# lynet55/robotic-mpc

Measured on AMD Instinct MI355X. Metric: MPC-steps/sec (whole node), UR10 N=100 dt=0.01 batch; 1/2/4/8 GPU, higher is better.
Workload: dtype f64

## Files before the change

### robotic_mpc_amd/csrc/mpc_core.h

```cpp
#pragma once
#include "mpc_kin.h"
#include "mpc_ipm.h"
#include "mpc_nlp.h"

#define MPC_REP16(X) X(0) X(1) X(2) X(3) X(4) X(5) X(6) X(7) X(8) X(9) X(10) X(11) X(12) X(13) X(14) X(15)
#define MPC_REP4(X) X(0) X(1) X(2) X(3)

namespace mpcb {

constexpr double BOUND_INF = 1e29;

constexpr int L1 = 98;
constexpr int L2N = 62;
constexpr int L2W = 114;

#ifndef MPCB_FUSE
#define MPCB_FUSE 1
#endif
#ifdef MPCB_PROFILE
#define PROF_T0(v) const double v = ex.clock()
#define PROF_ADD(i, v) prof[i] += ex.clock() - v
#else
#define PROF_T0(v)
#define PROF_ADD(i, v)
// ... 591 lines not shown
                        }
                    });
                }
                ex.par([&](int lane) {
                    ex.put_max(sm.red[0], lane, a_s.at(lane)); ex.put_max(sm.red[1], lane, a_e.at(lane));
                    ex.put_max(sm.red[2], lane, a_i.at(lane)); ex.put_max(sm.red[3], lane, a_c.at(lane));
                });
                rs = fmax(rs, ex.get_max(sm.red[0]));
                re = fmax(re, ex.get_max(sm.red[1]));
                ri = fmax(ri, ex.get_max(sm.red[2]));
                rc = fmax(rc, ex.get_max(sm.red[3]));
            }
            copies([&](int lane, auto nl) {
                constexpr int NL = decltype(nl)::value;
                if (wide) copy_lanes<W2, 0, W2, L2W, false, NL>(v2, ex.smem().w.G2, k0, k1, lane);
                else copy_lanes<W2_LIN, 0, W2, L2N, false, NL>(v2, ex.smem().w.G2, k0, k1, lane);
            });
            PROF_ADD(PF_X3, tn);
        }
        if (res4) { res4[0] = rs; res4[1] = re; res4[2] = ri; res4[3] = rc; }
        PROF_ADD(PF_NLP, t0);
        return cost;
    }

    MPC_PASS void residual_direct(int mode, double a)
    {
        PROF_T0(t0);
        Smem &sm = ex.smem();
        const InstParams &P = sm.P;
        const int Nl = ex.uni(ex.smem().n_hor), NS = Nl + 1;
        double *const G1 = ex.smem().w.G1, *const G2 = ex.smem().w.G2, *const G3 = ex.smem().w.G3;
        double *const Y = ex.pool();
        a = ex.uni(a);
        typename Ex::template PerLane<double> n_g, n_b, n_d, n_m, n_mu, n_c;
        PROF_T0(tx);
        ex.wpar([&](int lane) { n_g.at(lane) = 0; n_b.at(lane) = 0; n_d.at(lane) = 0; n_m.at(lane) = 0; n_mu.at(lane) = 0; n_c.at(lane) = 0; });
        if (mode == 1) {
            constexpr int IPS = 15, R = rounds_for(IPS);
            const int items = NS * IPS;
            for (int base = 0; base < items; base += R * NT) {
                ex.wpar([&](int lane) {
                    D2 cur[R], stp[R];
#pragma unroll
                    for (int r = 0; r < R; r++) {
                        const int e = imin(base + r * NT + lane, items - 1), k = e / IPS, c = 2 * (e - k * IPS);
                        cur[r] = *(MPC_GLOBAL const D2 *)(G1 + (size_t)k * W1 + O_QW + c);
                        stp[r] = *(MPC_GLOBAL const D2 *)(G3 + (size_t)(c >= 18 ? imin(k + 1, Nl) : k) * W3 + O_DW + c);
                    }
#pragma unroll
                    for (int r = 0; r < R; r++) {
                        const int e = base + r * NT + lane;
                        if (e < items) {
                            const int k = e / IPS, c = 2 * (e - k * IPS);
                            const double aa = (c >= 18 && k >= Nl) ? 0.0 : a;
                            D2 v = cur[r];
                            v.x += aa * stp[r].x; v.y += aa * stp[r].y;
                            *(MPC_GLOBAL D2 *)(G1 + (size_t)k * W1 + O_QW + c) = v;
                        }
                    }
                });
            }
        } else {
            ex.wpar([&](int lane) {
                if (lane < NX) gst(G1 + O_QW + 6 + lane, sm.xhat[lane] - gld(G1 + O_X + lane));
                if (lane >= 16 && lane < 16 + NU) gst(G1 + (size_t)Nl * W1 + O_QW + lane - 16, 0.0);
            });
        }
        {
            constexpr int IPS = 24, R = rounds_for(IPS);
            const int items = NS * IPS;
            for (int base = 0; base < items; base += R * NT) {
                ex.wpar([&](int lane) {
                    D2 cur[R], stp[R];
#pragma unroll
                    for (int r = 0; r < R; r++) {
                        const int e = imin(base + r * NT + lane, items - 1), k = e / IPS, q = 2 * (e - k * IPS);
                        cur[r] = *(MPC_GLOBAL const D2 *)(G1 + (size_t)k * W1 + O_QLAM + q);
                        if (mode == 1) stp[r] = *(MPC_GLOBAL const D2 *)(G3 + (size_t)k * W3 + O_DLAM + q);
                    }
                    double ncl = n_c.at(lane);
#pragma unroll
                    for (int r = 0; r < R; r++) {
                        const int e = base + r * NT + lane;
                        if (e < items) {
                            const int k = e / IPS, q = 2 * (e - k * IPS);
                            const bool is_t = q >= 24;
                            const int sc = is_t ? q - 24 : q, j = sc < 12 ? sc : sc - 12;
                            const bool ok = j < 6 ? k < Nl : (k >= 1 && k < Nl);
                            const D2 m = *reinterpret_cast<const D2 *>(&sm.bon[sc]);
                            const bool on0 = ok && m.x != 0.0, on1 = ok && m.y != 0.0;
                            D2 v = cur[r];
                            if (mode == 1) {
                                v.x = ipm::step_floor(on0, v.x, a, stp[r].x); v.y = ipm::step_floor(on1, v.y, a, stp[r].y);
                            } else {
                                v.x = is_t ? ipm::warm_t(on0, v.x) : ipm::warm_lam(on0, v.x);
                                v.y = is_t ? ipm::warm_t(on1, v.y) : ipm::warm_lam(on1, v.y);
                                ncl += (on0 && !is_t ? 1.0 : 0.0) + (on1 && !is_t ? 1.0 : 0.0);
                            }
                            *(MPC_GLOBAL D2 *)(G1 + (size_t)k * W1 + O_QLAM + q) = v;
                        }
                    }
                    n_c.at(lane) = ncl;
                });
            }
        }
        ex.barrier();
        PROF_ADD(PF_X1, tx);
        PROF_T0(ty);
        const int CY = ex.uni(imax(1, imin(ex.smem().pool_n / 6, NS)));
        for (int y0 = 0; y0 < NS; y0 += CY) {
        const int y1 = imin(y0 + CY, NS);
        if (y0 > 0) ex.barrier();
        {
            constexpr int R = rounds_for(NTASK);
            const int items = (imin(y1, Nl) - y0) * NTASK;
            for (int base = 0; base < items; base += R * NT) {
                ex.wpar([&](int lane) {
                    double g[R][12], d[R][12], rr[R];
#pragma unroll
                    for (int r = 0; r < R; r++) {
                        const int e = imax(imin(base + r * NT + lane, items - 1), 0), k = y0 + e / NTASK, i = e - (k - y0) * NTASK;
                        const double *g1 = G1 + (size_t)k * W1 + O_QW, *g2 = G2 + (size_t)k * W2;
                        rr[r] = gld(g2 + O_R + i);
#pragma unroll
                        for (int j = 0; j < 6; j++) { g[r][j] = gld(g2 + O_GQ + i * 6 + j); d[r][j] = gld(g1 + 6 + j); }
                        if (i == 4) {
#pragma unroll
                            for (int j = 0; j < 6; j++) { g[r][6 + j] = gld(g2 + O_GV + j); d[r][6 + j] = gld(g1 + 12 + j); }
                        }
                    }
#pragma unroll
                    for (int r = 0; r < R; r++) {
                        const int e = base + r * NT + lane;
                        if (e < items) {
                            const int k = y0 + e / NTASK, i = e - (k - y0) * NTASK;
                            double v = rr[r];
#pragma unroll
                            for (int j = 0; j < 6; j++) v += g[r][j] * d[r][j];
                            if (i == 4) {
#pragma unroll
                                for (int j = 0; j < 6; j++) v += g[r][6 + j] * d[r][6 + j];
                            }
                            v *= P.w_task[i];
                            Y[(k - y0) * 6 + i] = v;
                            gst(G2 + (size_t)k * W2 + O_Y + i, v);
                        }
                    }
                });
            }
        }
        ex.barrier();
        PROF_ADD(PF_X2, ty);
        PROF_T0(tz);
        {
            constexpr int R = Ex::VGPR_BUDGET <= 256 && rounds_for(6) > 2 ? 2 : rounds_for(6);
            const int items = (y1 - y0) * 6;
            const double dt = P.dt, lm = P.lm;
            auto bounds = [&](int lane, int k, int ci, double val_, double dv, double l_lo, double l_hi, double t_lo, double t_hi,
                              double &rg) {
                const bool hc = ci < 6 ? k < Nl : (k >= 1 && k < Nl);
                const bool blo = hc && sm.bon[ci] != 0.0, bhi = hc && sm.bon[12 + ci] != 0.0;
                const double val = hc ? val_ : 0.0;
                const double ll = blo ? l_lo : 0.0, lu = bhi ? l_hi : 0.0;
                const double itl = fast_rcp(t_lo), itu = fast_rcp(t_hi);
                const double rdl = blo ? dv - (bnd_lo(P, ci) - val) - t_lo : 0.0;
                const double rdu = bhi ? (bnd_hi(P, ci) - val) - dv - t_hi : 0.0;
                const double rml = ll * t_lo, rmu = lu * t_hi;
                double gt = rg;
                rg -= ll; gt -= ll;
                double gam = ll * itl;
                gt += (rml + ll * rdl) * itl;
                rg += lu; gt += lu;
                gam += lu * itu;
                gt -= (rmu + lu * rdu) * itu;
                n_mu.at(lane) += rml + rmu;
                n_d.at(lane) = fmax(n_d.at(lane), fmax(fabs(rdl), fabs(rdu)));
                n_m.at(lane) = fmax(n_m.at(lane), fmax(fabs(rml), fabs(rmu)));
                double *g3 = G3 + (size_t)k * W3, *g2 = G2 + (size_t)k * W2;
                gst(g3 + O_RD + ci, rdl); gst(g3 + O_RD + 12 + ci, rdu);
                gst(g3 + O_RM + ci, rml); gst(g3 + O_RM + 12 + ci, rmu);
                gst(g2 + O_GAM + ci, gam);
                return gt;
            };
            constexpr int RD = 2 * R;
            const int items_d = (y1 - y0) * NX;
            for (int base = 0; base < items; base += R * NT) {
                ex.wpar([&](int lane) {
                    double v[R][12], q[R][13], d[RD][5];
#pragma unroll
                    for (int r = 0; r < R; r++) {
                        const int e = imin(base + r * NT + lane, items - 1), k = y0 + e / 6, j = e - (k - y0) * 6, km = imax(k - 1, 0);
                        const double *g1 = G1 + (size_t)k * W1, *g2 = G2 + (size_t)k * W2, *gm = G1 + (size_t)km * W1;
                        v[r][0] = gld(g1 + O_U + j);      v[r][1] = gld(g1 + O_X + 6 + j);
                        v[r][2] = gld(g1 + O_QW + j);     v[r][3] = gld(g1 + O_QW + 12 + j);
                        v[r][4] = gld(g1 + O_QPI + j);    v[r][5] = gld(g1 + O_QPI + 6 + j);
                        v[r][6] = gld(gm + O_QPI + 6 + j);
                        v[r][7] = gld(g2 + O_GV + j);
                        v[r][8] = gld(g1 + O_QLAM + j);   v[r][9] = gld(g1 + O_QLAM + 12 + j);
                        v[r][10] = gld(g1 + O_QT + j);    v[r][11] = gld(g1 + O_QT + 12 + j);
                        q[r][0] = gld(g1 + O_X + j);  q[r][1] = gld(g1 + O_QW + 6 + j);
#pragma unroll
                        for (int i = 0; i < NTASK; i++) q[r][2 + i] = gld(g2 + O_GQ + i * 6 + j);
                        q[r][7] = v[r][4]; q[r][8] = gld(gm + O_QPI + j);
                        q[r][9] = gld(g1 + O_QLAM + 6 + j);  q[r][10] = gld(g1 + O_QLAM + 18 + j);
                        q[r][11] = gld(g1 + O_QT + 6 + j);   q[r][12] = gld(g1 + O_QT + 18 + j);
                    }
#pragma unroll
                    for (int r = 0; r < RD; r++) {
                        const int e = imin(2 * base + r * NT + lane, items_d - 1), k = y0 + e / NX, i = e - (k - y0) * NX, kn = imin(k + 1, Nl);
                        const double *dw = G1 + (size_t)k * W1 + O_QW;
                        d[r][0] = gld(dw + 6 + i);
                        d[r][1] = gld(dw + (i < 6 ? 12 + i : i - 6));
                        d[r][2] = gld(dw + (i < 6 ? i : i - 6));
                        d[r][3] = gld(G2 + (size_t)k * W2 + O_BD + i);
                        d[r][4] = gld(G1 + (size_t)kn * W1 + O_QW + 6 + i);
                    }
#pragma unroll
                    for (int r = 0; r < R; r++) {
                        const int e = base + r * NT + lane;
                        if (e < items) {
                            const int k = y0 + e / 6, j = e - (k - y0) * 6;
                            const double du = v[r][2], dvv = v[r][3];
                            const double uj = v[r][0] + du, vj = v[r][1] + dvv;
                            const double c2 = P.w_qddot * P.cq[j] * P.cq[j];
                            double *g3 = G3 + (size_t)k * W3, *g2 = G2 + (size_t)k * W2;
                            double rgu = 0.0;
                            if (k < Nl) {
                                rgu = dt * (2.0 * P.w_u * uj + c2 * (uj - vj));
                                rgu += P.b1[j] * v[r][4] + P.b2[j] * v[r][5];
                                rgu += dt * lm * du;
                            }
                            const double gtu = bounds(lane, k, j, v[r][0], du, v[r][8], v[r][9], v[r][10], v[r][11], rgu);
                            gst(g3 + O_RG + j, rgu); gst(g2 + O_GT + j, gtu);
                            double rgv = 0.0;
                            if (k >= 1) {
                                if (k < Nl) {
                                    rgv = dt * (v[r][7] * Y[(k - y0) * 6 + 4] + c2 * (vj - uj));
                                    rgv += P.a12[j] * v[r][4] + P.a22[j] * v[r][5];
                                }
                                rgv += (k < Nl ? dt : 1.0) * lm * dvv;
                                rgv -= v[r][6];
                            }
                            gst(g3 + O_RG + 12 + j, rgv); gst(g2 + O_GT + 12 + j, rgv);
                            const double dq = q[r][1];
                            double rg = 0.0;
                            if (k >= 1) {
                                if (k < Nl) {
                                    double s_ = 0.0;
#pragma unroll
                                    for (int i = 0; i < NTASK; i++) s_ += q[r][2 + i] * Y[(k - y0) * 6 + i];
                                    rg = dt * s_ + q[r][7];
                                }
                                rg += (k < Nl ? dt : 1.0) * lm * dq;
                                rg -= q[r][8];
                            }
                            const double gt = bounds(lane, k, 6 + j, q[r][0], dq, q[r][9], q[r][10], q[r][11], q[r][12], rg);
                            gst(g3 + O_RG + 6 + j, rg); gst(g2 + O_GT + 6 + j, gt);
                            n_g.at(lane) = fmax(n_g.at(lane), fmax(fmax(fabs(rgu), fabs(rgv)), fabs(rg)));
                        }
                    }
#pragma unroll
                    for (int r = 0; r < RD; r++) {
                        const int e = 2 * base + r * NT + lane;
                        if (e < items_d && e < 2 * (base + R * NT)) {
                            const int k = y0 + e / NX, i = e - (k - y0) * NX;
                            double vv = 0.0;
                            if (k < Nl) {
                                if (i < 6) vv = d[r][0] + P.a12[i] * d[r][1] + P.b1[i] * d[r][2];
                                else vv = P.a22[i - 6] * d[r][0] + P.b2[i - 6] * d[r][1];
                                vv += d[r][3] - d[r][4];
                                n_b.at(lane) = fmax(n_b.at(lane), fabs(vv));
                            }
                            gst(G2 + (size_t)k * W2 + O_RB + i, vv);
                        }
                    }
                });
            }
        }
        PROF_ADD(PF_X3, tz);
        }
        ex.par([&](int lane) {
            ex.put_max(sm.red[0], lane, n_g.at(lane)); ex.put_max(sm.red[1], lane, n_b.at(lane));
            ex.put_max(sm.red[2], lane, n_d.at(lane)); ex.put_max(sm.red[3], lane, n_m.at(lane));
            ex.put_sum(sm.red[4], lane, n_mu.at(lane)); ex.put_sum(sm.red[5], lane, n_c.at(lane));
        });
        const double ng = ex.get_max(sm.red[0]), nb = ex.get_max(sm.red[1]), nd = ex.get_max(sm.red[2]), nm = ex.get_max(sm.red[3]);
        const double smu = ex.get_sum(sm.red[4]), nc = ex.get_sum(sm.red[5]);
        ex.par([&](int lane) {
            if ((lane & (WAVE - 1)) == 0) {
                sm.ret[0] = ng; sm.ret[1] = nb; sm.ret[2] = nd; sm.ret[3] = nm; sm.ret[4] = smu;
                if (mode == 0) sm.ret[5] = nc;
            }
        });
        PROF_ADD(PF_RES, t0);
    }

    struct FactLane {
        double b1a, b2a, b1b, b2b, a12a, a22a, a12b, a22b;
        double hu_c;
        double huv_c;
        double lm_c;
        double mqq, mqv, mvq, mvv;
        double qqq, qqv, qvq, qvv;
        int a, b;
        int oqq, oqv, ovv;
    };

    template <int MODE>
    MPC_PASS void fact_pass_t()
    {
        constexpr bool RES = MODE == 1, SEG = MODE == 2;
        PROF_T0(t0);
        Smem &sm = ex.smem();
        const InstParams &P = sm.P;
        const int Nl = ex.uni(ex.smem().n_hor);
        constexpr int WR = 78;
        constexpr int WF = RES ? W4 - O_PM : W4;
        constexpr int FO = RES ? O_PM : 0;
        const ResMap rm = res_map();
        const int CH = RES ? chunk_len_in(rm.scr_n, 2 * (WR + WF), 2 * WR) : chunk_len(2 * (WR + W4), 2 * WR);
        typename Ex::template PerLane<FactLane> fl;
        ex.seq([&](int lane) {
            FactLane &f = fl.at(lane);
            const int a = lane < 36 ? lane / 6 : 0, b = lane < 36 ? lane % 6 : 0;
            f.a = a; f.b = b;
            f.oqq = tri(imin(a, b), imax(a, b)); f.oqv = tri(a, 6 + b); f.ovv = tri(6 + imin(a, b), 6 + imax(a, b));
            f.b1a = P.b1[a]; f.b2a = P.b2[a]; f.b1b = P.b1[b]; f.b2b = P.b2[b];
            f.a12a = P.a12[a]; f.a22a = P.a22[a]; f.a12b = P.a12[b]; f.a22b = P.a22[b];
            const double c2 = P.dt * P.w_qddot * P.cq[a] * P.cq[a];
            f.hu_c = a == b ? P.dt * 2.0 * P.w_u + c2 + P.dt * P.lm : 0.0;
            f.huv_c = a == b ? c2 : 0.0;
            f.lm_c = a == b ? P.dt * P.lm : 0.0;
            f.mqq = f.mqv = f.mvq = f.mvv = 0.0;
            f.qqq = f.qqv = f.qvq = f.qvv = 0.0;
        });
        const double dw0 = P.dt * P.w_task[0], dw1 = P.dt * P.w_task[1], dw2 = P.dt * P.w_task[2], dw3 = P.dt * P.w_task[3],
                     dw4 = P.dt * P.w_task[4];
        auto next_stage = [&](int lane, FactLane &f, double gam_u, int sb) {
            const double fq = f.b1a * f.mqq + f.b2a * f.mvq, fv = f.b1a * f.mqv + f.b2a * f.mvv;
            double r = fq * f.b1b + fv * f.b2b + f.hu_c;
            r += f.a == f.b ? gam_u : 0.0;
            sm.Rt[f.a * 6 + f.b] = r;
            double *St = sm.St2[sb];
            St[f.a * 12 + f.b] = fq;
            St[f.a * 12 + 6 + f.b] = fq * f.a12b + fv * f.a22b - f.huv_c;
            const double cq = f.a12a * f.mqq + f.a22a * f.mvq, cv = f.a12a * f.mqv + f.a22a * f.mvv;
            f.qqq = f.mqq;
            f.qqv = f.mqq * f.a12b + f.mqv * f.a22b;
            f.qvq = cq;
            f.qvv = cq * f.a12b + cv * f.a22b;
            (void)lane;
        };
        int sb = 0;
        const size_t buf = (size_t)(CH + 1) * WR + (size_t)CH * WF;
        auto vr_of = [&](int ci) { return ex.pool() + (size_t)(ci & 1) * buf; };
        auto vf_of = [&](int ci) { return vr_of(ci) + (size_t)(CH + 1) * WR; };
        auto k1_of = [&](int ci) { return Nl - ci * CH; };
        typename Ex::template PerLane<double> pr;
        typename Ex::template PerLane<double> tr, wr;
        typename Ex::template PerLane<D2> ab;
        double b1r[6], b2r[6], a12r[6], a22r[6];
#pragma unroll
        for (int i = 0; i < 6; i++) { b1r[i] = P.b1[i]; b2r[i] = P.b2[i]; a12r[i] = P.a12[i]; a22r[i] = P.a22[i]; }
        typename Ex::template PerLane<double> phi[12];
        int vcur = 0;
        auto vec_sweep = [&](int ci) {
            const int k1c = k1_of(ci), k0c = imax(k1c - CH + 1, 0), klc = imax(k0c - 1, 0);
            const double *vr = vr_of(ci);
            double *vf = vf_of(ci);
            for (int k = k1c; k >= k0c; k--) {
                const double *ric = vr + (size_t)(k - klc) * WR;
                const double *gt = ric + 48, *rbv = ric + 66;
                double *fac = vf + (size_t)(k - k0c) * WF - FO;
                double *kk = RES ? rm.K + (size_t)k * 72 : fac + O_K, *vhp = RES ? rm.VH + (size_t)k * 6 : fac + O_VH;
                double *ep = RES ? rm.E + (size_t)k * 12 : fac + O_E, *pvp = RES ? rm.P + (size_t)k * 12 : fac + O_PV;
                const double *Pn = (k < k1c ? fac + WF : vf_of(ci + 1) - FO) + O_PM;
                const int vnxt = vcur ^ 1;
                ex.await(&sm.prog, Nl - k);
                if (k == Nl) {
                    ex.sub([&](int lane) {
                        if (lane < NX) {
                            const double v = gt[6 + lane];
                            pr.at(lane) = v; ex.share(sm.pv[vcur], lane, v);
                            pvp[lane] = v; fac[O_WV + lane] = 0.0; ep[lane] = 0.0;
                            const int j = lane % 6;
                            D2 c2; c2.x = P.a12[j]; c2.y = P.a22[j];
                            ab.at(lane) = c2;
                        }
                        if (lane < NU) vhp[lane] = 0.0;
                        if (lane == 0) ex.post(&sm.prog1, 0);
                    });
                    continue;
                }
                ex.sub([&](int lane) {
                    double t = 0.0, w = 0.0;
                    if (lane < NX) {
                        double w0 = 0.0, w1 = 0.0;
#pragma unroll
                        for (int j = 0; j < NX; j += 2) { w0 += Pn[tri_sym(lane, j)] * rbv[j]; w1 += Pn[tri_sym(lane, j + 1)] * rbv[j + 1]; }
                        w = w0 + w1;
                        t = pr.at(lane) + w;
                    }
                    tr.at(lane) = t; wr.at(lane) = w;
                    ex.share(sm.mt2[vcur], lane < NX ? lane : NX, t);
                });
                ex.sub([&](int lane) {
                    const double t = tr.at(lane), w = wr.at(lane);
                    double tv[12];
#pragma unroll
                    for (int i = 0; i < NX; i++) tv[i] = ex.gather(sm.mt2[vcur], i, t);
                    const double oq = ex.shr6(sm.mt2[vcur], lane, t);
                    if (lane < NX) {
                        const int j = lane;
                        double hu[6];
#pragma unroll
                        for (int m = 0; m < 6; m++) hu[m] = gt[m] + b1r[m] * tv[m] + b2r[m] * tv[6 + m];
                        const D2 c2 = ab.at(lane);
                        double pj = gt[6 + j] + (j < 6 ? t : c2.x * oq + c2.y * t);
                        double s0 = 0.0, s1 = 0.0;
#pragma unroll
                        for (int m = 0; m < 6; m += 2) { s0 += kk[m * 12 + j] * hu[m]; s1 += kk[(m + 1) * 12 + j] * hu[m + 1]; }
                        pj -= s0 + s1;
                        pr.at(lane) = pj; ex.share(sm.pv[vnxt], lane, pj);
                        pvp[j] = pj;
                        fac[O_WV + j] = w;
                        const int i6 = j < 6 ? j : j - 6;
                        double v0 = 0.0, v1 = 0.0;
#pragma unroll
                        for (int m = 0; m < 6; m += 2) { v0 += fac[O_RI + i6 * 6 + m] * hu[m]; v1 += fac[O_RI + i6 * 6 + m + 1] * hu[m + 1]; }
                        const double vh = v0 + v1;
                        if (j < 6) vhp[j] = vh;
                        ep[j] = rbv[j] - (j < 6 ? P.b1[i6] : P.b2[i6]) * vh;
                    }
                    if (lane == 0) ex.post(&sm.prog1, Nl - k);
                });
                vcur = vnxt;
            }
        };
        constexpr int NBW = Ex::BG_WAVES;
        ex.par([&](int lane) {
            if (lane == 0) { ex.post(&sm.prog, -1); ex.post(&sm.prog1, -1); ex.post(&sm.flg[0], NBW); ex.post(&sm.flg[1], 0); }
        });
        load_rect<WR, O_GQ, W2>(vr_of(0), ex.smem().w.G2, imax(imax(Nl - CH + 1, 0) - 1, 0), Nl);
        const int nwin = (Nl + CH) / CH;
        PROF_T0(ts);
        ex.pipeline3(nwin, [&](int ci) {
            const int k1 = k1_of(ci), k0 = imax(k1 - CH + 1, 0), kl = imax(k0 - 1, 0);
            double *vr = vr_of(ci), *vf = vf_of(ci);
            ex.await(&sm.flg[0], NBW * (ci + 1));
            if (ci >= 2) ex.await(&sm.flg[1], NBW * ci);
            for (int k = k1; k >= k0; k--) {
                const double *ric = vr + (size_t)(k - kl) * WR;
                const double *ricd = ric - WR;
                double *fac = vf + (size_t)(k - k0) * WF - FO;
                double *kk = RES ? rm.K + (size_t)k * 72 : fac + O_K;
                const double *gam = ric + 36;
                if (k == Nl) {
                    ex.seq([&](int lane) {
                        const double lmN = ex.smem().P.lm;
                        for (int e = lane; e < NPM; e += WAVE) {
                            double v = 0.0;
#pragma unroll
                            for (int i = 0; i < NX; i++) v = e == tri(i, i) ? lmN : v;
                            fac[O_PM + e] = v;
                        }
                        if (lane < 36) {
                            FactLane &f = fl.at(lane);
                            f.mqv = f.mvq = 0.0;
                            f.mqq = f.mvv = f.a == f.b ? lmN : 0.0;
                            next_stage(lane, f, ricd[36 + f.a], sb);
                        }
                        if (lane == 0) ex.post(&sm.prog, 0);
                    });
                    continue;
                }
#ifndef MPCB_DIAG_NO_B
                ex.seq([&](int lane) {
                    const double *St = sm.St2[sb];
                    double A_[6][6];
#pragma unroll
                    for (int i = 0; i < 6; i++)
#pragma unroll
                        for (int j = 0; j <= i; j++) A_[i][j] = sm.Rt[i * 6 + j];
                    double dinv[6];
#pragma unroll
                    for (int j = 0; j < 6; j++) {
#ifdef MPCB_DIAG_NO_LDL
                        dinv[j] = A_[j][j]; continue;
#endif
                        dinv[j] = fast_rcp(A_[j][j]);
                        double lj[6];
#pragma unroll
                        for (int i = j + 1; i < 6; i++) lj[i] = A_[i][j] * dinv[j];
#pragma unroll
                        for (int i = j + 1; i < 6; i++)
#pragma unroll
                            for (int r = j + 1; r <= i; r++) A_[i][r] -= lj[i] * A_[r][j];
#pragma unroll
                        for (int i = j + 1; i < 6; i++) A_[i][j] = lj[i];
                    }
                    if (lane < 18) {
                        double x[6];
                        const int col = lane < 12 ? lane : 0;
#pragma unroll
                        for (int i = 0; i < 6; i++) x[i] = St[i * 12 + col];
#pragma unroll
                        for (int i = 0; i < 6; i++) x[i] = lane < 12 ? x[i] : (i == lane - 12 ? 1.0 : 0.0);
#pragma unroll
                        for (int j = 0; j < 6; j++) {
#pragma unroll
                            for (int i = j + 1; i < 6; i++) x[i] -= A_[i][j] * x[j];
                        }
#pragma unroll
                        for (int i = 0; i < 6; i++) x[i] *= dinv[i];
#pragma unroll
                        for (int j = 5; j >= 0; j--) {
#pragma unroll
                            for (int i = 0; i < j; i++) x[i] -= A_[j][i] * x[j];
                        }
                        if (lane < 12) {
#pragma unroll
                            for (int i = 0; i < 6; i++) kk[i * 12 + lane] = x[i];
                        } else {
#pragma unroll
                            for (int i = 0; i < 6; i++) fac[O_RI + i * 6 + (lane - 12)] = x[i];
                        }
                    }
                });
#endif
                ex.seq([&](int lane) {
#ifdef MPCB_DIAG_NO_CA
                    if (lane == 0) ex.post(&sm.prog, Nl - k);
                    return;
#endif
                    if (lane < 36) {
                        FactLane &f = fl.at(lane);
                        if (k > 0) {
                            const double *St = sm.St2[sb];
                            const double *gq = ric, *gv = ric + 30;
                            const double ga0 = gq[f.a], ga1 = gq[6 + f.a], ga2 = gq[12 + f.a], ga3 = gq[18 + f.a], ga4 = gq[24 + f.a];
                            const double gb0 = gq[f.b], gb1 = gq[6 + f.b], gb2 = gq[12 + f.b], gb3 = gq[18 + f.b], gb4 = gq[24 + f.b];
                            const double gva = gv[f.a], gvb = gv[f.b];
                            const double gam_q = gam[6 + f.a], gam_u = ricd[36 + f.a];
                            double sa[6], sva[6], kb[6], kvb[6];
#pragma unroll
                            for (int m = 0; m < 6; m++) { sa[m] = St[m * 12 + f.a]; sva[m] = St[m * 12 + 6 + f.a]; }
#pragma unroll
                            for (int m = 0; m < 6; m++) { kb[m] = kk[m * 12 + f.b]; kvb[m] = kk[m * 12 + 6 + f.b]; }
#if defined(__HIP_DEVICE_COMPILE__)
                            asm volatile("" ::: "memory");
#endif
                            double pqq = f.qqq + (dw0 * ga0 * gb0 + dw1 * ga1 * gb1 + dw2 * ga2 * gb2 + dw3 * ga3 * gb3 + dw4 * ga4 * gb4) + f.lm_c;
                            double pqv = f.qqv + dw4 * ga4 * gvb;
                            double pvq = f.qvq + dw4 * gva * gb4;
                            double pvv = f.qvv + dw4 * gva * gvb + (f.huv_c + f.lm_c);
                            pqq += f.a == f.b ? gam_q : 0.0;
#pragma unroll
                            for (int m = 0; m < 6; m++) {
                                pqq -= sa[m] * kb[m]; pqv -= sa[m] * kvb[m];
                                pvq -= sva[m] * kb[m]; pvv -= sva[m] * kvb[m];
                            }
                            f.mqq = pqq; f.mqv = pqv; f.mvq = pvq; f.mvv = pvv;
                            next_stage(lane, f, gam_u, sb ^ 1);
                            if (f.a <= f.b) { fac[O_PM + f.oqq] = pqq; fac[O_PM + f.ovv] = pvv; }
                            fac[O_PM + f.oqv] = pqv;
                        }
                    }
                    if (lane == 0) ex.post(&sm.prog, Nl - k);
                });
                sb ^= 1;
            }
            }, [&](int ci) {
#ifndef MPCB_DIAG_NO_VEC
                vec_sweep(ci);
#endif
            }, [&](int ci, int lane, auto nl) {
                constexpr int NL = decltype(nl)::value;
                const int k1 = k1_of(ci), k0 = imax(k1 - CH + 1, 0);
                const int nk1 = k0 - 1, nk0 = imax(nk1 - CH + 1, 0), nkl = imax(nk0 - 1, 0);
                const int pk1 = k1 + CH, pk0 = k1 + 1;
                if (ci > 0) ex.await(&sm.prog1, Nl - pk0);
                if (nk1 >= 0) copy_lanes<WR, O_GQ, W2, WR, true, NL>(vr_of(ci + 1), ex.smem().w.G2, nkl, nk1, lane);
                if ((lane & (WAVE - 1)) == 0) ex.post_add(&sm.flg[0], 1);
                if (ci > 0) copy_lanes<WF, FO, W4, WF, false, NL>(vf_of(ci - 1), ex.smem().w.G4, pk0, pk1, lane);
                ex.await(&sm.prog1, Nl - k1);
                if ((lane & (WAVE - 1)) == 0) ex.post_add(&sm.flg[1], 1);
                if constexpr (RES || SEG) {
#ifndef MPCB_DIAG_NO_PHI
                    if (lane < WAVE) {
                        const int L = SEG ? (reg_ok() ? RL : seg_map().L) : rm.L;
                        for (int k = imin(k1, Nl - 1); k >= k0; k--) {
                            ex.await(&sm.prog, Nl - k);
                            const double *kk = RES ? rm.K + (size_t)k * 72 : vf_of(ci) + (size_t)(k - k0) * WF - FO + O_K;
                            const int c = k / L;
                            const bool first = ex.uni(k == imin((c + 1) * L, Nl) - 1), last = ex.uni(k == c * L);
                            const D2 kv2 = reinterpret_cast<const D2 *>(kk)[(lane & (WAVE - 1)) < 36 ? (lane & (WAVE - 1)) : 0];
                            auto Kat = [&](int idx) { return ex.lane_value(kk, idx, (idx & 1) ? kv2.y : kv2.x, idx >> 1); };
                            {
                                double ph[12], g[6], nw[12];
#pragma unroll
                                for (int j = 0; j < 12; j++) ph[j] = first ? (j == lane ? 1.0 : 0.0) : phi[j].at(lane);
#pragma unroll
                                for (int m = 0; m < 6; m++) g[m] = ph[m] * b1r[m] + ph[6 + m] * b2r[m];
#pragma unroll
                                for (int j = 0; j < 6; j++) {
                                    double s0 = ph[j], s1 = a12r[j] * ph[j] + a22r[j] * ph[6 + j];
#pragma unroll
                                    for (int m = 0; m < 6; m++) { s0 -= g[m] * Kat(m * 12 + j); s1 -= g[m] * Kat(m * 12 + 6 + j); }
                                    nw[j] = s0; nw[6 + j] = s1;
                                }
#pragma unroll
                                for (int j = 0; j < 12; j++) phi[j].at(lane) = nw[j];
                                if (last && lane < NX) {
                                    if (SEG) {
#pragma unroll
                                        for (int j = 0; j < 12; j++) gst(ex.smem().w.PH + (size_t)c * 144 + lane * 12 + j, nw[j]);
                                    } else {
#pragma unroll
                                        for (int j = 0; j < 12; j++) rm.PHI[(size_t)c * 144 + lane * 12 + j] = nw[j];
                                    }
                                }
                            }
                        }
                    }
#endif
                }
            });
        PROF_ADD(PF_SEQ_FACT, ts);
        {
            const int k1 = k1_of(nwin - 1);
            copy_rect<WF, FO, W4, WF, false>(vf_of(nwin - 1), ex.smem().w.G4, 0, k1);
        }
        PROF_ADD(PF_FACT, t0);
    }

    MPC_PASS void corrector_bwd_pass(double sigma_mu)
    {
        PROF_T0(t0);
        Smem &sm = ex.smem();
        const InstParams &P = sm.P;
        const int Nl = ex.uni(ex.smem().n_hor);
        constexpr int WLT = 50;
        constexpr int L3 = 90;
        constexpr int C_DLAM = 42, C_DT = 66;
        constexpr int WGR = 30;
        constexpr int WK = 72, WW = 50;
        constexpr int WC = 12;
        constexpr int WRM = 24, WHP = 30;
        constexpr int C_PV = 18;
        constexpr int PER = WLT + L3 + WGR + WK + WW + WC + WRM + WHP;
        const int CH = chunk_len(2 * PER, 0);
        typename Ex::template PerLane<D2> ab;
        typename Ex::template PerLane<double> pr;
        double b1r[6], b2r[6];
#pragma unroll
        for (int i = 0; i < 6; i++) { b1r[i] = P.b1[i]; b2r[i] = P.b2[i]; }
        ex.seq([&](int lane) {
            const int j = lane % 6;
            D2 v; v.x = P.a12[j]; v.y = P.a22[j];
            ab.at(lane) = v;
            pr.at(lane) = 0.0;
        });
        auto carve = [&](int sel, double *&vlt, double *&v3, double *&vgr, double *&vk, double *&vw, double *&vc, double *&orm,
                         double *&ohp) {
            vlt = ex.pool() + (size_t)sel * CH * PER;
            v3 = vlt + (size_t)CH * WLT; vgr = v3 + (size_t)CH * L3; vk = vgr + (size_t)CH * WGR;
            vw = vk + (size_t)CH * WK; vc = vw + (size_t)CH * WW; orm = vc + (size_t)CH * WC; ohp = orm + (size_t)CH * WRM;
        };
        int cur = 0, bsel = 0;
        {
            double *vlt, *v3, *vgr, *vk, *vw, *vc, *orm, *ohp;
            carve(0, vlt, v3, vgr, vk, vw, vc, orm, ohp);
            const int f0 = imax(Nl - CH + 1, 0);
            copies([&](int lane, auto nl) {
                constexpr int NL = decltype(nl)::value;
                copy_lanes<48, O_QLAM, W1, WLT, true, NL>(vlt, ex.smem().w.G1, f0, Nl, lane);
                copy_lanes<42, 0, W3, L3, true, NL>(v3, ex.smem().w.G3, f0, Nl, lane);
                copy_lanes<48, O_DLAM, W3, L3, true, NL>(v3 + C_DLAM, ex.smem().w.G3, f0, Nl, lane);
                copy_lanes<WGR, O_GT, W2, WGR, true, NL>(vgr, ex.smem().w.G2, f0, Nl, lane);
                copy_lanes<WK, O_K, W4, WK, true, NL>(vk, ex.smem().w.G4, f0, Nl, lane);
                copy_lanes<48, O_WV, W4, WW, true, NL>(vw, ex.smem().w.G4, f0, Nl, lane);
            });
        }
        for (int k1 = Nl; k1 >= 0; k1 -= CH, bsel ^= 1) {
            const int k0 = imax(k1 - CH + 1, 0);
            double *vlt, *v3, *vgr, *vk, *vw, *vc, *orm, *ohp;
            carve(bsel, vlt, v3, vgr, vk, vw, vc, orm, ohp);
            double *nlt, *n3, *ngr, *nk, *nw, *nc_, *prm, *php;
            carve(bsel ^ 1, nlt, n3, ngr, nk, nw, nc_, prm, php);
            const int nk1 = k0 - 1, nk0 = imax(nk1 - CH + 1, 0);
            ex.par([&](int lane) {
                const int rows = k1 - k0 + 1;
                for (int e = lane; e < rows * NB; e += NT) {
                    const int s = e / NB, j = e - s * NB, k = k0 + s;
                    const double *lt = vlt + (size_t)s * WLT;
                    const double *r3 = v3 + (size_t)s * L3;
                    double *rmo = orm + (size_t)s * WRM;
                    const bool hc = has_comp(Nl, k, j);
                    const bool blo = hc && bnd_lo(P, j) > -BOUND_INF, bhi = hc && bnd_hi(P, j) < BOUND_INF;
                    const double ll = lt[j], tl = lt[24 + j], lu = lt[12 + j], tu = lt[36 + j];
                    const double dll = r3[C_DLAM + j], dtl = r3[C_DT + j], dlu = r3[C_DLAM + 12 + j], dtu = r3[C_DT + 12 + j];
                    const double rdl = r3[18 + j], rdu = r3[18 + 12 + j];
                    double gt = r3[j];
                    double rml, rmu;
                    gt += ipm::corrector_side(blo, ll, tl, dll, dtl, rdl, sigma_mu, rml);
                    gt -= ipm::corrector_side(bhi, lu, tu, dlu, dtu, rdu, sigma_mu, rmu);
                    if (hc) vgr[(size_t)s * WGR + j] = gt;
                    rmo[j] = rml; rmo[12 + j] = rmu;
                }
            });
            ex.par([&](int lane) {
                const int rows = k1 - k0 + 1;
                for (int e = lane; e < rows * NX; e += NT) {
                    const int s = e / NX, j = e - s * NX, k = k0 + s;
                    const double *gt = vgr + (size_t)s * WGR, *w = vw + (size_t)s * WW, *kf = vk + (size_t)s * WK;
                    double v = 0.0;
                    if (k < Nl) {
                        v = gt[6 + j] + (j < 6 ? w[j] : P.a12[j - 6] * w[j - 6] + P.a22[j - 6] * w[j]);
#pragma unroll
                        for (int m = 0; m < 6; m++) v -= kf[m * 12 + j] * (gt[m] + P.b1[m] * w[m] + P.b2[m] * w[6 + m]);
                    }
                    vc[(size_t)s * WC + j] = v;
                }
            });
            PROF_T0(ts);
            ex.overlap([&]() {
            for (int k = k1; k >= k0; k--) {
                const double *gt = vgr + (size_t)(k - k0) * WGR;
                const double *cv = vc + (size_t)(k - k0) * WC;
                const double *kf = vk + (size_t)(k - k0) * WK;
                double *hp = ohp + (size_t)(k - k0) * WHP;
                const int nxt = cur ^ 1;
                if (k == Nl) {
                    ex.seq([&](int lane) {
                        if (lane < NX) {
                            const double v = gt[6 + lane];
                            pr.at(lane) = v; ex.share(sm.pv[cur], lane, v);
                            hp[C_PV + lane] = v;
                            hp[6 + lane] = 0.0;
                        }
                        if (lane < NU) hp[lane] = 0.0;
                    });
                    continue;
                }
                ex.seq([&](int lane) {
                    const int jc = lane < NX ? lane : 0;
                    double kc[6];
#pragma unroll
                    for (int i = 0; i < 6; i++) kc[i] = kf[i * 12 + jc];
                    const double ck = cv[jc];
                    const double mine = pr.at(lane);
                    double pn[12];
#pragma unroll
                    for (int i = 0; i < NX; i++) pn[i] = ex.gather(sm.pv[cur], i, mine);
                    const double oq = ex.shr6(sm.pv[cur], lane, mine);
                    double acc0 = 0.0, acc1 = 0.0;
#pragma unroll
                    for (int i = 0; i < 6; i += 2) {
                        acc0 += kc[i] * (b1r[i] * pn[i] + b2r[i] * pn[6 + i]);
                        acc1 += kc[i + 1] * (b1r[i + 1] * pn[i + 1] + b2r[i + 1] * pn[7 + i]);
                    }
                    const D2 c2 = ab.at(lane);
                    const double at = lane < 6 ? mine : c2.x * oq + c2.y * mine;
                    const double pj = ck + (at - (acc0 + acc1));
                    pr.at(lane) = pj;
                    if (lane < NX) {
                        ex.share(sm.pv[nxt], lane, pj);
                        hp[C_PV + lane] = pj;
                    }
                });
                cur = nxt;
            }
            }, [&](int lane, auto nl) {
                constexpr int NL = decltype(nl)::value;
                if (nk1 >= 0) {
                    copy_lanes<48, O_QLAM, W1, WLT, true, NL>(nlt, ex.smem().w.G1, nk0, nk1, lane);
                    copy_lanes<42, 0, W3, L3, true, NL>(n3, ex.smem().w.G3, nk0, nk1, lane);
                    copy_lanes<48, O_DLAM, W3, L3, true, NL>(n3 + C_DLAM, ex.smem().w.G3, nk0, nk1, lane);
                    copy_lanes<WGR, O_GT, W2, WGR, true, NL>(ngr, ex.smem().w.G2, nk0, nk1, lane);
                    copy_lanes<WK, O_K, W4, WK, true, NL>(nk, ex.smem().w.G4, nk0, nk1, lane);
                    copy_lanes<48, O_WV, W4, WW, true, NL>(nw, ex.smem().w.G4, nk0, nk1, lane);
                }
                if (k1 < Nl) {
                    copy_lanes<WRM, O_RM, W3, WRM, false, NL>(prm, ex.smem().w.G3, k1 + 1, k1 + CH, lane);
                    copy_lanes<WHP, O_VH, W4, WHP, false, NL>(php, ex.smem().w.G4, k1 + 1, k1 + CH, lane);
                }
            });
            PROF_ADD(PF_SEQ_BWD, ts);
            ex.par([&](int lane) {
                const int rows = k1 - k0 + 1;
                for (int e = lane; e < rows * NX; e += NT) {
                    const int s = e / NX, j = e - s * NX, k = k0 + s;
                    if (k >= Nl) continue;
                    const double *gt = vgr + (size_t)s * WGR, *w = vw + (size_t)s * WW, *ri = w + 12;
                    const double *pn = (s + 1 < rows ? ohp + (size_t)(s + 1) * WHP : php) + C_PV;
                    const int i6 = j < 6 ? j : j - 6;
                    double v0 = 0.0, v1 = 0.0;
#pragma unroll
                    for (int m = 0; m < 6; m += 2) {
                        const double h0 = gt[m] + P.b1[m] * (pn[m] + w[m]) + P.b2[m] * (pn[6 + m] + w[6 + m]);
                        const double h1 = gt[m + 1] + P.b1[m + 1] * (pn[m + 1] + w[m + 1]) + P.b2[m + 1] * (pn[7 + m] + w[7 + m]);
                        v0 += ri[i6 * 6 + m] * h0; v1 += ri[i6 * 6 + m + 1] * h1;
                    }
                    const double vh = v0 + v1;
                    double *hp = ohp + (size_t)s * WHP;
                    if (j < 6) hp[j] = vh;
                    hp[6 + j] = gt[18 + j] - (j < 6 ? P.b1[i6] : P.b2[i6]) * vh;
                }
            });
            if (k0 == 0) {
                copies([&](int lane, auto nl) {
                    constexpr int NL = decltype(nl)::value;
                    copy_lanes<WRM, O_RM, W3, WRM, false, NL>(orm, ex.smem().w.G3, k0, k1, lane);
                    copy_lanes<WHP, O_VH, W4, WHP, false, NL>(ohp, ex.smem().w.G4, k0, k1, lane);
                });
            }
        }
        PROF_ADD(PF_BWD, t0);
    }

    template <bool AFFINE, bool FAST = false>
    MPC_PASS double forward_step_pass()
    {
        static_assert(!FAST || !AFFINE, "the fast path takes the full step");
        PROF_T0(t0);
        Smem &sm = ex.smem();
        const InstParams &P = sm.P;
        const int Nl = ex.uni(ex.smem().n_hor);
        constexpr int WLT = 50, WR = 50, WO = 78;
        constexpr int LF = AFFINE ? W4_AFF : W4_FWD;
        constexpr int PER = LF + WLT + WR + WO;
#ifndef MPCB_FWD_BLK
#define MPCB_FWD_BLK 4
#endif
        constexpr int BLK = MPCB_FWD_BLK;
        const int CH = chunk_len(2 * PER, 0);
        const int NCH = (Nl + CH) / CH;
        double *const pool = ex.pool();
        typename Ex::template PerLane<D2> ab, bb;
        typename Ex::template PerLane<double> dxr;
        typename Ex::template PerLane<double> r_al, r_a0, r_a1, r_a2;
        ex.par([&](int lane) {
            const int j = (lane & (WAVE - 1)) % 6;
            D2 v; v.x = P.a12[j]; v.y = P.a22[j];
            ab.at(lane) = v;
            D2 u; u.x = P.b1[j]; u.y = P.b2[j];
            bb.at(lane) = u;
            dxr.at(lane) = 0.0;
            if (lane < NX) ex.share(sm.dx[0], lane, 0.0);
            r_al.at(lane) = 1.0; r_a0.at(lane) = 0.0; r_a1.at(lane) = 0.0; r_a2.at(lane) = 0.0;
            if (lane == 0) ex.post(&sm.prog, -1);
        });
        int cur = 0;
        {
            double *q4 = pool, *qlt = q4 + (size_t)CH * LF, *qr = qlt + (size_t)CH * WLT;
            const int e1 = imin(CH - 1, Nl);
            copies([&](int lane, auto nl) {
                constexpr int NL = decltype(nl)::value;
                copy_lanes<LF, 0, W4, LF, true, NL>(q4, ex.smem().w.G4, 0, e1, lane);
                if (FAST) copy_lanes<18, 0, W1, WLT, true, NL>(qlt, ex.smem().w.G1, 0, e1, lane);
                else {
                copy_lanes<48, O_QLAM, W1, WLT, true, NL>(qlt, ex.smem().w.G1, 0, e1, lane);
                copy_lanes<48, O_RD, W3, WR, true, NL>(qr, ex.smem().w.G3, 0, e1, lane);
                }
            });
        }
        for (int ci = 0; ci < NCH; ci++) {
            const int k0 = ci * CH, k1 = imin(k0 + CH - 1, Nl);
            double *v4 = pool + (size_t)(ci & 1) * CH * PER;
// ... 1373 lines not shown
```

Baseline: 1.559 million.

## Keep LDL solve results in per-lane registers instead of round-tripping through kk

Measured after the change: 1.476 million. 0.947x the previous value.

```diff
diff --git a/robotic_mpc_amd/csrc/mpc_core.h b/robotic_mpc_amd/csrc/mpc_core.h
--- a/robotic_mpc_amd/csrc/mpc_core.h
+++ b/robotic_mpc_amd/csrc/mpc_core.h
@@ -917,9 +917,21 @@
         double lm_c;
         double mqq, mqv, mvq, mvv;
         double qqq, qqv, qvq, qvv;
+        double kb[6], kvb[6];
         int a, b;
         int oqq, oqv, ovv;
     };
+
+    template <int MODE>
+    MPC_HD int fact_chunk() const
+    {
+        constexpr int WR = 78, WF = MODE == 1 ? W4 - O_PM : W4;
+        return MODE == 1 ? chunk_len_in(res_map().scr_n, 2 * (WR + WF), 2 * WR) : chunk_len(2 * (WR + W4), 2 * WR);
+    }
+    template <class E>
+    MPC_HD static auto fact_probe(E &e, double *kk, int k, int) -> decltype(e.fact_probe(kk, k), void()) { e.fact_probe(kk, k); }
+    template <class E>
+    MPC_HD static void fact_probe(E &, double *, int, long) {}
 
     template <int MODE>
     MPC_PASS void fact_pass_t()
@@ -933,7 +945,7 @@
         constexpr int WF = RES ? W4 - O_PM : W4;
         constexpr int FO = RES ? O_PM : 0;
         const ResMap rm = res_map();
-        const int CH = RES ? chunk_len_in(rm.scr_n, 2 * (WR + WF), 2 * WR) : chunk_len(2 * (WR + W4), 2 * WR);
+        const int CH = fact_chunk<MODE>();
         typename Ex::template PerLane<FactLane> fl;
         ex.seq([&](int lane) {
             FactLane &f = fl.at(lane);
@@ -948,6 +960,8 @@
             f.lm_c = a == b ? P.dt * P.lm : 0.0;
             f.mqq = f.mqv = f.mvq = f.mvv = 0.0;
             f.qqq = f.qqv = f.qvq = f.qvv = 0.0;
+#pragma unroll
+            for (int i = 0; i < 6; i++) f.kb[i] = f.kvb[i] = 0.0;
         });
         const double dw0 = P.dt * P.w_task[0], dw1 = P.dt * P.w_task[1], dw2 = P.dt * P.w_task[2], dw3 = P.dt * P.w_task[3],
                      dw4 = P.dt * P.w_task[4];
@@ -1114,35 +1128,31 @@
 #pragma unroll
                         for (int i = j + 1; i < 6; i++) A_[i][j] = lj[i];
                     }
-                    if (lane < 18) {
-                        double x[6];
-                        const int col = lane < 12 ? lane : 0;
-#pragma unroll
-                        for (int i = 0; i < 6; i++) x[i] = St[i * 12 + col];
-#pragma unroll
-                        for (int i = 0; i < 6; i++) x[i] = lane < 12 ? x[i] : (i == lane - 12 ? 1.0 : 0.0);
+                    if (lane < 42) {
+                        FactLane &f = fl.at(lane);
+                        double x[6], y[6];
+#pragma unroll
+                        for (int i = 0; i < 6; i++) { x[i] = St[i * 12 + f.b]; y[i] = St[i * 12 + 6 + f.b]; }
+#pragma unroll
+                        for (int i = 0; i < 6; i++) x[i] = lane < 36 ? x[i] : (i == lane - 36 ? 1.0 : 0.0);
 #pragma unroll
                         for (int j = 0; j < 6; j++) {
 #pragma unroll
-                            for (int i = j + 1; i < 6; i++) x[i] -= A_[i][j] * x[j];
-                        }
-#pragma unroll
-                        for (int i = 0; i < 6; i++) x[i] *= dinv[i];
+                            for (int i = j + 1; i < 6; i++) { x[i] -= A_[i][j] * x[j]; y[i] -= A_[i][j] * y[j]; }
+                        }
+#pragma unroll
+                        for (int i = 0; i < 6; i++) { x[i] *= dinv[i]; y[i] *= dinv[i]; }
 #pragma unroll
                         for (int j = 5; j >= 0; j--) {
 #pragma unroll
-                            for (int i = 0; i < j; i++) x[i] -= A_[j][i] * x[j];
-                        }
-                        if (lane < 12) {
-#pragma unroll
-                            for (int i = 0; i < 6; i++) kk[i * 12 + lane] = x[i];
-                        } else {
-#pragma unroll
-                            for (int i = 0; i < 6; i++) fac[O_RI + i * 6 + (lane - 12)] = x[i];
-                        }
+                            for (int i = 0; i < j; i++) { x[i] -= A_[j][i] * x[j]; y[i] -= A_[j][i] * y[j]; }
+                        }
+#pragma unroll
+                        for (int i = 0; i < 6; i++) { f.kb[i] = x[i]; f.kvb[i] = y[i]; }
                     }
                 });
 #endif
+                fact_probe(ex, kk, k, 0);
                 ex.seq([&](int lane) {
 #ifdef MPCB_DIAG_NO_CA
                     if (lane == 0) ex.post(&sm.prog, Nl - k);
@@ -1157,11 +1167,10 @@
                             const double gb0 = gq[f.b], gb1 = gq[6 + f.b], gb2 = gq[12 + f.b], gb3 = gq[18 + f.b], gb4 = gq[24 + f.b];
                             const double gva = gv[f.a], gvb = gv[f.b];
                             const double gam_q = gam[6 + f.a], gam_u = ricd[36 + f.a];
-                            double sa[6], sva[6], kb[6], kvb[6];
+                            double sa[6], sva[6];
 #pragma unroll
                             for (int m = 0; m < 6; m++) { sa[m] = St[m * 12 + f.a]; sva[m] = St[m * 12 + 6 + f.a]; }
-#pragma unroll
-                            for (int m = 0; m < 6; m++) { kb[m] = kk[m * 12 + f.b]; kvb[m] = kk[m * 12 + 6 + f.b]; }
+                            const double *kb = f.kb, *kvb = f.kvb;
 #if defined(__HIP_DEVICE_COMPILE__)
                             asm volatile("" ::: "memory");
 #endif
@@ -1180,6 +1189,14 @@
                             if (f.a <= f.b) { fac[O_PM + f.oqq] = pqq; fac[O_PM + f.ovv] = pvv; }
                             fac[O_PM + f.oqv] = pqv;
                         }
+                        if (f.a == 0) {
+#pragma unroll
+                            for (int i = 0; i < 6; i++) { kk[i * 12 + f.b] = f.kb[i]; kk[i * 12 + 6 + f.b] = f.kvb[i]; }
+                        }
+                    } else if (lane < 42) {
+                        const FactLane &f = fl.at(lane);
+#pragma unroll
+                        for (int i = 0; i < 6; i++) fac[O_RI + i * 6 + (lane - 36)] = f.kb[i];
                     }
                     if (lane == 0) ex.post(&sm.prog, Nl - k);
                 });
```
